# feiyeha/EGM-Unet

Measured on AMD Instinct MI355X. Metric: train images/sec at 3x512x512 bs=8/GPU, higher is better.
Workload: dtype bf16; 1 GPU; EGM-UNet GRFBUNet(3,2,base_c=32) fwd+5-term-loss+bwd+SGD, 8x3x512x512 per GPU (BASELINE.json configs[1]); global_batch=8, parallelism=dp1, launch=hipGraph replay, world_size=1

## Files before the change

### egm_unet_amd/csrc/mca.hip

```cpp
#include "common.h"
#include "bn_elem.h"
#include <stdlib.h>

namespace {

inline int stream_grid(long long total_threads) {
    long long b = (total_threads + 255) / 256;
    if (b > 256 * 16) b = 256 * 16;
    if (b < 1) b = 1;
    return (int)b;
}
__device__ __forceinline__ float sigm(float v) { return 1.f / (1.f + expf(-v)); }

template <typename T, int MODE>
__global__ __launch_bounds__(256) void mca_reduce_row_kernel(const T* __restrict__ a, int lda, const T* __restrict__ b, int ldb,
                                                             float* __restrict__ sums, float* __restrict__ colp, float* __restrict__ chp,
                                                             int H, int W, int C, const float* __restrict__ scale = nullptr,
                                                             const float* __restrict__ shift = nullptr, int act = 0,
                                                             T* __restrict__ zout = nullptr, int ldz = 0) {
    __shared__ float st[2 * 256 * 8];
    __shared__ float red[16];
    const int n = blockIdx.y, h = blockIdx.x, tid = threadIdx.x, ncv = C >> 3, slots = 256 / ncv;
    const int cv = tid % ncv, slot = tid / ncv, L = H + W + C;
    const long long rowbase = ((long long)n * H + h) * W;
    float s8[8], q8[8], ts = 0.f, tq = 0.f;
    zero8(s8); zero8(q8);
    float sc8[8], sh8[8];
    if (MODE == 2) {
#pragma unroll
        for (int j = 0; j < 8; ++j) { sc8[j] = scale[cv * 8 + j]; sh8[j] = shift[cv * 8 + j]; }
    }
    for (int w0 = 0; w0 < W; w0 += slots) {
        const int w = w0 + slot;
        float ps = 0.f, pq = 0.f;
        if (w < W) {
            float v[8];
            load8(a + (rowbase + w) * lda + cv * 8, v);
            if (MODE == 1) {
                float u[8];
                load8(b + (rowbase + w) * ldb + cv * 8, u);
#pragma unroll
                for (int j = 0; j < 8; ++j) v[j] *= u[j];
            }
            if (MODE == 2) {
#pragma unroll
                for (int j = 0; j < 8; ++j) v[j] = to_f32(from_f32<T>(bn_fwd_elem<sizeof(T) == 2>(v[j], sc8[j], sh8[j], act)));
                store8(zout + (rowbase + w) * ldz + cv * 8, v);
            }
#pragma unroll
            for (int j = 0; j < 8; ++j) { s8[j] += v[j]; q8[j] += v[j] * v[j]; ps += v[j]; pq += v[j] * v[j]; }
        }
        ts += ps; tq += pq;
        for (int o = ncv >> 1; o > 0; o >>= 1) { ps += __shfl_xor(ps, o, 64); pq += __shfl_xor(pq, o, 64); }
        if (w < W && cv == 0) { colp[(rowbase + w) * 2 + 0] = ps; colp[(rowbase + w) * 2 + 1] = pq; }
    }
#pragma unroll
    for (int j = 0; j < 8; ++j) { st[tid * 8 + j] = s8[j]; st[(256 + tid) * 8 + j] = q8[j]; }
    __syncthreads();
    for (int c = tid; c < C; c += 256) {
        float cs = 0.f, cq = 0.f;
        for (int sl = 0; sl < slots; ++sl) { cs += st[(sl * ncv + (c >> 3)) * 8 + (c & 7)]; cq += st[(256 + sl * ncv + (c >> 3)) * 8 + (c & 7)]; }
        chp[(((long long)n * H + h) * C + c) * 2 + 0] = cs;
        chp[(((long long)n * H + h) * C + c) * 2 + 1] = cq;
    }
    ts = block_sum(ts, red);
    tq = block_sum(tq, red);
    if (tid == 0) { sums[((long long)n * L + h) * 2 + 0] = ts; sums[((long long)n * L + h) * 2 + 1] = tq; }
}
__global__ __launch_bounds__(256) void mca_reduce_h_kernel(const float* __restrict__ colp, const float* __restrict__ chp, float* __restrict__ sums,
                                                           int N, int H, int W, int C) {
    __shared__ double red[256];
    const int L = H + W + C, per_img = (W + C) * 2;
    const int n = blockIdx.y, col = threadIdx.x & 15, hl = threadIdx.x >> 4;
    const int f = blockIdx.x * 16 + col;
    double s = 0.0;
    if (f < per_img) {
        const bool is_col = f < W * 2;
        const float* src = is_col ? colp + (long long)n * H * W * 2 + f : chp + (long long)n * H * C * 2 + (f - W * 2);
        const int pitch = is_col ? W * 2 : C * 2;
        for (int h = hl; h < H; h += 16) s += (double)src[(long long)h * pitch];
    }
    red[threadIdx.x] = s;
    __syncthreads();
    if (hl == 0 && f < per_img) {
        double t = 0.0;
        for (int j = 0; j < 16; ++j) t += red[j * 16 + col];
        sums[((long long)n * L + H) * 2 + f] = (float)t;
    }
}

struct GateParams {
    const float* w[3];
    const float* k[3];
    int ks[3];
    float inv;
};
__device__ __forceinline__ void axis_of(int e, int H, int W, int C, int& ax, int& idx, int& len) {
    const int L = H + W + C, r = e % L;
    if (r < H) { ax = 0; idx = r; len = H; } else if (r < H + W) { ax = 1; idx = r - H; len = W; } else { ax = 2; idx = r - H - W; len = C; }
}
__device__ __forceinline__ float axis_count(int ax, int H, int W, int C) {
    return ax == 0 ? (float)C * (float)W : (ax == 1 ? (float)C * (float)H : (float)H * (float)W);
}
template <bool LDS_O>
__global__ void mca_gates_fwd_kernel(const float* __restrict__ sums, GateParams gp, float* __restrict__ stats, float* __restrict__ o,
                                     float* __restrict__ gates, int N, int H, int W, int C) {
    extern __shared__ float gate_lds[];
    const int L = H + W + C, total = N * L;
    __shared__ float sk[3][8], sab[3][2];
    if (threadIdx.x < 24) { const int a = threadIdx.x >> 3, t = threadIdx.x & 7; sk[a][t] = t < gp.ks[a] ? gp.k[a][t] : 0.f; }
    else if (threadIdx.x >= 32 && threadIdx.x < 38) { const int a = (threadIdx.x - 32) >> 1, j = (threadIdx.x - 32) & 1; sab[a][j] = gp.ks[a] > 0 ? 0.5f + sigm(gp.w[a][j]) : 0.f; }
    __syncthreads();
    for (int e = threadIdx.x; e < total; e += blockDim.x) {
        int ax, idx, len; axis_of(e, H, W, C, ax, idx, len);
        const double cnt = (double)axis_count(ax, H, W, C);
        const double S = sums[e * 2], Q = sums[e * 2 + 1];
        const double mean = S / cnt;
        double var = (Q - S * S / cnt) / (cnt - 1.0);
        if (var < 0.0) var = 0.0;
        const float sd = (float)sqrt(var);
        stats[e * 2] = (float)mean; stats[e * 2 + 1] = sd;
        const float ov = sab[ax][0] * (float)mean + sab[ax][1] * sd;
        o[e] = ov;
        if (LDS_O) gate_lds[e] = ov;
    }
    __syncthreads();
    const float* os = LDS_O ? gate_lds : o;
    for (int e = threadIdx.x; e < total; e += blockDim.x) {
        int ax, idx, len; axis_of(e, H, W, C, ax, idx, len);
        const int ks = gp.ks[ax], pad = (ks - 1) / 2;
        float z = 0.f;
        for (int t = 0; t < ks; ++t) { const int j = idx + t - pad; if (j >= 0 && j < len) z += sk[ax][t] * os[e - idx + j]; }
        gates[e] = ks > 0 ? sigm(z) : 0.f;
    }
}
template <bool LDS_IN>
__global__ void mca_gates_bwd_kernel(const float* __restrict__ dG, const float* __restrict__ stats, const float* __restrict__ o,
                                     const float* __restrict__ gates, GateParams gp, float* __restrict__ dz, float* __restrict__ coef,
                                     float* __restrict__ dwts, float* __restrict__ dks, int N, int H, int W, int C) {
    extern __shared__ float gate_lds[];
    const int L = H + W + C, total = N * L;
    if (LDS_IN) {
        float* sdz = gate_lds; float* so = gate_lds + total; float* sst = gate_lds + 2 * total;
        for (int e = threadIdx.x; e < total; e += blockDim.x) {
            sdz[e] = dG[e * 2] * gp.inv * gates[e] * (1.f - gates[e]);
            so[e] = o[e];
            sst[2 * e] = stats[2 * e]; sst[2 * e + 1] = stats[2 * e + 1];
        }
        dz = sdz; o = so; stats = sst;
    }
    __shared__ float sk[3][8], sab[3][2];
    if (threadIdx.x < 24) { const int a = threadIdx.x >> 3, t = threadIdx.x & 7; sk[a][t] = t < gp.ks[a] ? gp.k[a][t] : 0.f; }
    else if (threadIdx.x >= 32 && threadIdx.x < 38) { const int a = (threadIdx.x - 32) >> 1, j = (threadIdx.x - 32) & 1; sab[a][j] = gp.ks[a] > 0 ? 0.5f + sigm(gp.w[a][j]) : 0.f; }
    if (threadIdx.x >= 64 && threadIdx.x < 64 + 24) dks[threadIdx.x - 64] = 0.f;
    if (!LDS_IN)
        for (int e = threadIdx.x; e < total; e += blockDim.x) dz[e] = dG[e * 2] * gp.inv * gates[e] * (1.f - gates[e]);
    __syncthreads();
    float acc[27];
#pragma unroll
    for (int i = 0; i < 27; ++i) acc[i] = 0.f;
    for (int e = threadIdx.x; e < total; e += blockDim.x) {
        int ax, idx, len; axis_of(e, H, W, C, ax, idx, len);
        const int ks = gp.ks[ax], pad = (ks - 1) / 2;
        float d_o = 0.f;
        for (int t = 0; t < ks; ++t) { const int i = idx - t + pad; if (i >= 0 && i < len) d_o += sk[ax][t] * dz[e - idx + i]; }
        const float alpha = sab[ax][0], beta = sab[ax][1];
        const float mean = stats[e * 2], sd = stats[e * 2 + 1];
        const float cnt = axis_count(ax, H, W, C);
        const float dmean = alpha * d_o, dsd = beta * d_o;
        const float B = sd > 0.f ? dsd / ((cnt - 1.f) * sd) : 0.f;
        coef[e * 2] = dmean / cnt - B * mean; coef[e * 2 + 1] = B;
        const float dze = dz[e];
#pragma unroll
        for (int a = 0; a < 3; ++a)
            if (a == ax) {
                acc[a * 2] += d_o * mean; acc[a * 2 + 1] += d_o * sd;
#pragma unroll
                for (int t = 0; t < 7; ++t) {
                    const int j = idx + t - pad;
                    if (t < ks && j >= 0 && j < len) acc[6 + a * 7 + t] += dze * o[e - idx + j];
                }
            }
    }
    __shared__ float part[16][27];
    const int lane = threadIdx.x & 63, wv = threadIdx.x >> 6, nw = (blockDim.x + 63) >> 6;
#pragma unroll
    for (int i = 0; i < 27; ++i) { const float v = wave_sum(acc[i]); if (lane == 0) part[wv][i] = v; }
    __syncthreads();
    if (threadIdx.x < 27) {
        float v = 0.f;
        for (int w = 0; w < nw; ++w) v += part[w][threadIdx.x];
        const int i = threadIdx.x;
        if (i < 6) {
            const float sg = gp.ks[i >> 1] > 0 ? sigm(gp.w[i >> 1][i & 1]) : 0.f;
            dwts[i] = v * sg * (1.f - sg);
        } else {
            const int a = (i - 6) / 7, t = (i - 6) % 7;
            if (t < gp.ks[a]) dks[a * 8 + t] = v;
        }
    }
}

template <typename T>
__global__ void mca_xout_kernel(const T* __restrict__ x, int ldx, const float* __restrict__ gates, T* __restrict__ xo, int ldo, int N, int H,
                                int W, int C, float inv) {
    const int ncv = C >> 3, L = H + W + C;
    const long long total = (long long)N * H * W * ncv;
    for (long long i = blockIdx.x * 256LL + threadIdx.x; i < total; i += (long long)gridDim.x * 256) {
        long long p; int cv; egm_divmod(i, ncv, p, cv);
        int w, h, n; egm_pix_nyx(p, H, W, n, h, w);
        const float* g = gates + (long long)n * L;
        const float ghw = g[h] + g[H + w];
        float v[8];
        load8(x + p * ldx + cv * 8, v);
#pragma unroll
        for (int j = 0; j < 8; ++j) v[j] *= (ghw + g[H + W + cv * 8 + j]) * inv;
        store8(xo + p * ldo + cv * 8, v);
    }
}
__device__ __forceinline__ int shuffle_src(int c, int C) { return (c & 3) * (C >> 2) + (c >> 2); }
__device__ __forceinline__ int shuffle_dst(int c, int C) { const int q = C >> 2; return (c % q) * 4 + c / q; }

template <typename T>
__global__ void mca_stencil1_kernel(const T* __restrict__ xo, int ld, T* __restrict__ r1, int ldr, T* __restrict__ u2, int ldu,
                                    unsigned char* __restrict__ codes, int N, int H, int W, int C) {
    const int ncv = C >> 3;
    const long long total = (long long)N * H * W * ncv;
    for (long long i = blockIdx.x * 256LL + threadIdx.x; i < total; i += (long long)gridDim.x * 256) {
        long long p; int cv; egm_divmod(i, ncv, p, cv);
        int xx, yy; egm_pix_yx(p, H, W, yy, xx);
        float c[8], mx[8], mn[8], s[8], v[8];
        int amx[8], amn[8];
        load8(xo + p * ld + cv * 8, c);
#pragma unroll
        for (int j = 0; j < 8; ++j) { mx[j] = -INFINITY; mn[j] = INFINITY; s[j] = 0.f; amx[j] = 4; amn[j] = 4; }
#pragma unroll
        for (int r = -1; r <= 1; ++r)
#pragma unroll
            for (int q = -1; q <= 1; ++q) {
                if (yy + r < 0 || yy + r >= H || xx + q < 0 || xx + q >= W) continue;
                load8(xo + (p + (long long)r * W + q) * ld + cv * 8, v);
#pragma unroll
                for (int j = 0; j < 8; ++j) {
                    if (v[j] > mx[j]) { mx[j] = v[j]; amx[j] = (r + 1) * 3 + (q + 1); }
                    if (v[j] < mn[j]) { mn[j] = v[j]; amn[j] = (r + 1) * 3 + (q + 1); }
                    s[j] += v[j];
                }
            }
        float o1[8], o2[8];
#pragma unroll
        for (int j = 0; j < 8; ++j) {
            const float sh = to_f32(xo[p * ld + shuffle_src(cv * 8 + j, C)]);
            o1[j] = 0.51f * c[j] + 0.2f * (mx[j] - mn[j]) + 0.1f * sh;
            const float u = c[j] - s[j] * (1.f / 9.f);
            o2[j] = u * u;
        }
        store8(r1 + p * ldr + cv * 8, o1); store8(u2 + p * ldu + cv * 8, o2);
        if (codes != nullptr) {
            uint2 cd;
            cd.x = (amx[0] | (amn[0] << 4)) | ((amx[1] | (amn[1] << 4)) << 8) | ((amx[2] | (amn[2] << 4)) << 16) | ((amx[3] | (amn[3] << 4)) << 24);
            cd.y = (amx[4] | (amn[4] << 4)) | ((amx[5] | (amn[5] << 4)) << 8) | ((amx[6] | (amn[6] << 4)) << 16) | ((amx[7] | (amn[7] << 4)) << 24);
            *reinterpret_cast<uint2*>(codes + p * C + cv * 8) = cd;
        }
    }
}
template <typename T>
__global__ void add_avg3_kernel(const T* __restrict__ a, int lda, const T* __restrict__ b, int ldb, float scale, T* __restrict__ out, int ldo,
                                int N, int H, int W, int C) {
    const int ncv = C >> 3;
    const long long total = (long long)N * H * W * ncv;
    for (long long i = blockIdx.x * 256LL + threadIdx.x; i < total; i += (long long)gridDim.x * 256) {
        long long p; int cv; egm_divmod(i, ncv, p, cv);
        int xx, yy; egm_pix_yx(p, H, W, yy, xx);
        float c[8], s[8], v[8];
        load8(a + p * lda + cv * 8, c);
        zero8(s);
#pragma unroll
        for (int r = -1; r <= 1; ++r)
#pragma unroll
            for (int q = -1; q <= 1; ++q) {
                if (yy + r < 0 || yy + r >= H || xx + q < 0 || xx + q >= W) continue;
                load8(b + (p + (long long)r * W + q) * ldb + cv * 8, v);
#pragma unroll
                for (int j = 0; j < 8; ++j) s[j] += v[j];
            }
#pragma unroll
        for (int j = 0; j < 8; ++j) c[j] += scale * s[j] * (1.f / 9.f);
        store8(out + p * ldo + cv * 8, c);
    }
}
constexpr int MF_TY = 16, MF_TX = 16, MF_CB = 32, MF_PY = MF_TY + 4, MF_PX = MF_TX + 4, MF_UY = MF_TY + 2, MF_UX = MF_TX + 2;
template <typename T>
__global__ __launch_bounds__(256) void mca_fused_fwd_kernel(const T* __restrict__ x, int ldx, const float* __restrict__ gates,
                                                            T* __restrict__ xo, int ldxo, T* __restrict__ out, int ldo,
                                                            unsigned char* __restrict__ codes, int N, int H, int W, int C, int tiles_x,
                                                            int tiles_y, int nchunk, float inv) {
    extern __shared__ __attribute__((aligned(16))) unsigned char mf_smem[];
    T* sxo = reinterpret_cast<T*>(mf_smem);
    T* su2 = sxo + MF_PY * MF_PX * MF_CB;
    const int tid = threadIdx.x, L = H + W + C;
    int b = xcd_contiguous_item(blockIdx.x, gridDim.x);
    const int chunk = b % nchunk; b /= nchunk;
    const int tx = b % tiles_x; b /= tiles_x;
    const int ty = b % tiles_y; const int n = b / tiles_y;
    const int y0 = ty * MF_TY, x0 = tx * MF_TX, c0 = chunk * MF_CB;
    const int nvec = (C - c0 < MF_CB ? C - c0 : MF_CB) >> 3;
    const float* __restrict__ g = gates + (long long)n * L;
    const long long img = (long long)n * H * W;
    __shared__ float sgh[MF_PY], sgw[MF_PX];
    if (tid < MF_PY) { const int gy = y0 + tid - 2; sgh[tid] = (gy >= 0 && gy < H) ? g[gy] : 0.f; }
    else if (tid >= 64 && tid < 64 + MF_PX) { const int gx = x0 + tid - 64 - 2; sgw[tid - 64] = (gx >= 0 && gx < W) ? g[H + gx] : 0.f; }
    const int vt = tid & 3;
    float gc8[8], gs8[8];
#pragma unroll
    for (int j = 0; j < 8; ++j) {
        const bool okv = vt < nvec;
        gc8[j] = okv ? g[H + W + c0 + vt * 8 + j] : 0.f;
        gs8[j] = okv ? g[H + W + shuffle_src(c0 + vt * 8 + j, C)] : 0.f;
    }

    constexpr int NC = MF_TY * MF_TX * 4 / 256;
    T shv[NC][8];
#pragma unroll
    for (int k = 0; k < NC; ++k) {
        const int i = tid + k * 256, pix = i >> 2, v = i & 3, ly = pix / MF_TX, lx = pix - ly * MF_TX;
        const int gy = y0 + ly, gx = x0 + lx;
        const bool ok = v < nvec && gy < H && gx < W;
        const long long p = img + (long long)(ok ? gy : 0) * W + (ok ? gx : 0);
        const int q0 = ok ? ((c0 + v * 8) >> 2) : 0;
#pragma unroll
        for (int grp = 0; grp < 4; ++grp) {
            const T* sp = x + p * ldx + (ok ? grp * (C >> 2) : 0) + q0;
            if (sizeof(T) == 2 && ((C >> 2) & 1) == 0) {
                const uint32_t two = *reinterpret_cast<const uint32_t*>(sp);
                __builtin_memcpy(&shv[k][grp], &two, 2);
                const uint16_t hi = (uint16_t)(two >> 16);
                __builtin_memcpy(&shv[k][grp + 4], &hi, 2);
            } else {
                shv[k][grp] = sp[0]; shv[k][grp + 4] = sp[1];
            }
        }
    }
    constexpr int NA = (MF_PY * MF_PX * 4 + 255) / 256;
    uint4 raw[NA];
#pragma unroll
    for (int k = 0; k < NA; ++k) {
        const int i = tid + k * 256, pix = i >> 2, v = i & 3, py = pix / MF_PX, px = pix - py * MF_PX;
        const int gy = y0 + py - 2, gx = x0 + px - 2;
        raw[k] = make_uint4(0, 0, 0, 0);
        if (i < MF_PY * MF_PX * 4 && v < nvec && gy >= 0 && gy < H && gx >= 0 && gx < W) {
            const T* src = x + (img + (long long)gy * W + gx) * ldx + c0 + v * 8;
            if (sizeof(T) == 2) raw[k] = *reinterpret_cast<const uint4*>(src);
        }
    }
    __syncthreads();
#pragma unroll
    for (int k = 0; k < NA; ++k) {
        const int i = tid + k * 256, pix = i >> 2, v = i & 3, py = pix / MF_PX, px = pix - py * MF_PX;
        const int gy = y0 + py - 2, gx = x0 + px - 2;
        if (i >= MF_PY * MF_PX * 4) continue;
        float val[8];
        zero8(val);
        if (v < nvec && gy >= 0 && gy < H && gx >= 0 && gx < W) {
            const long long p = img + (long long)gy * W + gx;
            if (sizeof(T) == 2) load8(reinterpret_cast<const T*>(&raw[k]), val);
            else load8(x + p * ldx + c0 + v * 8, val);
            const float ghw = sgh[py] + sgw[px];
#pragma unroll
            for (int j = 0; j < 8; ++j) val[j] = to_f32(from_f32<T>(val[j] * ((ghw + gc8[j]) * inv)));
            if (xo != nullptr && py >= 2 && py < MF_TY + 2 && px >= 2 && px < MF_TX + 2) store8(xo + p * ldxo + c0 + v * 8, val);
        }
        store8_lds(sxo + pix * MF_CB + v * 8, val);
    }
    __syncthreads();
    for (int i = tid; i < MF_UY * MF_UX * 4; i += 256) {
        const int pix = i >> 2, v = i & 3, uy = pix / MF_UX, ux = pix - uy * MF_UX;
        const int gy = y0 + uy - 1, gx = x0 + ux - 1;
        float o2[8];
        zero8(o2);
        if (v < nvec && gy >= 0 && gy < H && gx >= 0 && gx < W) {
            float c[8], s8[8], t[8];
            zero8(s8);
            const T* ctr = sxo + ((uy + 1) * MF_PX + ux + 1) * MF_CB + v * 8;
            load8(ctr, c);
#pragma unroll
            for (int r = -1; r <= 1; ++r)
#pragma unroll
                for (int q = -1; q <= 1; ++q) {
                    load8(ctr + (r * MF_PX + q) * MF_CB, t);
#pragma unroll
                    for (int j = 0; j < 8; ++j) s8[j] += t[j];
                }
#pragma unroll
            for (int j = 0; j < 8; ++j) { const float u = c[j] - s8[j] * (1.f / 9.f); o2[j] = u * u; }
        }
        store8_lds(su2 + pix * MF_CB + v * 8, o2);
    }
    __syncthreads();
#pragma unroll
    for (int k = 0; k < NC; ++k) {
        const int i = tid + k * 256;
        const int pix = i >> 2, v = i & 3, ly = pix / MF_TX, lx = pix - ly * MF_TX;
        const int gy = y0 + ly, gx = x0 + lx;
        if (v >= nvec || gy >= H || gx >= W) continue;
        const long long p = img + (long long)gy * W + gx;
        float c[8], mx[8], mn[8], t[8], s2[8];
        int amx[8], amn[8];
        const T* ctr = sxo + ((ly + 2) * MF_PX + lx + 2) * MF_CB + v * 8;
        const T* uctr = su2 + ((ly + 1) * MF_UX + lx + 1) * MF_CB + v * 8;
        load8(ctr, c);
        zero8(s2);
#pragma unroll
        for (int j = 0; j < 8; ++j) { mx[j] = -INFINITY; mn[j] = INFINITY; amx[j] = 4; amn[j] = 4; }
#pragma unroll
        for (int r = -1; r <= 1; ++r)
#pragma unroll
            for (int q = -1; q <= 1; ++q) {
                load8(uctr + (r * MF_UX + q) * MF_CB, t);
#pragma unroll
                for (int j = 0; j < 8; ++j) s2[j] += t[j];
                if (gy + r < 0 || gy + r >= H || gx + q < 0 || gx + q >= W) continue;
                load8(ctr + (r * MF_PX + q) * MF_CB, t);
#pragma unroll
                for (int j = 0; j < 8; ++j) {
                    if (t[j] > mx[j]) { mx[j] = t[j]; amx[j] = (r + 1) * 3 + (q + 1); }
                    if (t[j] < mn[j]) { mn[j] = t[j]; amn[j] = (r + 1) * 3 + (q + 1); }
                }
            }
        const float ghw = sgh[ly + 2] + sgw[lx + 2];
        float o[8];
#pragma unroll
        for (int j = 0; j < 8; ++j) {
            const float sh = to_f32(from_f32<T>(to_f32(shv[k][j]) * ((ghw + gs8[j]) * inv)));
            const float o1 = to_f32(from_f32<T>(0.51f * c[j] + 0.2f * (mx[j] - mn[j]) + 0.1f * sh));
            o[j] = o1 + 0.2f * s2[j] * (1.f / 9.f);
        }
        store8(out + p * ldo + c0 + v * 8, o);
        if (codes != nullptr) {
            uint2 cd;
            cd.x = (amx[0] | (amn[0] << 4)) | ((amx[1] | (amn[1] << 4)) << 8) | ((amx[2] | (amn[2] << 4)) << 16) | ((amx[3] | (amn[3] << 4)) << 24);
            cd.y = (amx[4] | (amn[4] << 4)) | ((amx[5] | (amn[5] << 4)) << 8) | ((amx[6] | (amn[6] << 4)) << 16) | ((amx[7] | (amn[7] << 4)) << 24);
            *reinterpret_cast<uint2*>(codes + p * C + c0 + v * 8) = cd;
        }
    }
}
template <typename T>
__global__ void mca_bwd_du_kernel(const T* __restrict__ xo, int ld, const T* __restrict__ g, int ldg, T* __restrict__ du, int ldd, int N, int H,
                                  int W, int C) {
    const int ncv = C >> 3;
    const long long total = (long long)N * H * W * ncv;
    for (long long i = blockIdx.x * 256LL + threadIdx.x; i < total; i += (long long)gridDim.x * 256) {
        long long p; int cv; egm_divmod(i, ncv, p, cv);
        int xx, yy; egm_pix_yx(p, H, W, yy, xx);
        float c[8], s[8], sg[8], v[8];
        load8(xo + p * ld + cv * 8, c);
        zero8(s); zero8(sg);
#pragma unroll
        for (int r = -1; r <= 1; ++r)
#pragma unroll
            for (int q = -1; q <= 1; ++q) {
                if (yy + r < 0 || yy + r >= H || xx + q < 0 || xx + q >= W) continue;
                load8(xo + (p + (long long)r * W + q) * ld + cv * 8, v);
#pragma unroll
                for (int j = 0; j < 8; ++j) s[j] += v[j];
                load8(g + (p + (long long)r * W + q) * ldg + cv * 8, v);
#pragma unroll
                for (int j = 0; j < 8; ++j) sg[j] += v[j];
            }
#pragma unroll
        for (int j = 0; j < 8; ++j) c[j] = 0.4f * (c[j] - s[j] * (1.f / 9.f)) * sg[j] * (1.f / 9.f);
        store8(du + p * ldd + cv * 8, c);
    }
}
template <typename T>
__global__ void mca_bwd_dxo_kernel(const unsigned char* __restrict__ codes, const T* __restrict__ g, int ldg, const T* __restrict__ du, int ldd,
                                   T* __restrict__ dxo, int ldo, int N, int H, int W, int C) {
    const int ncv = C >> 3;
    const long long total = (long long)N * H * W * ncv;
    for (long long i = blockIdx.x * 256LL + threadIdx.x; i < total; i += (long long)gridDim.x * 256) {
        long long p; int cv; egm_divmod(i, ncv, p, cv);
        int xx, yy; egm_pix_yx(p, H, W, yy, xx);
        float acc[8], sd[8], v[8], gp[8];
        zero8(acc); zero8(sd);
#pragma unroll
        for (int r = -1; r <= 1; ++r)
#pragma unroll
            for (int q = -1; q <= 1; ++q) {
                if (yy + r < 0 || yy + r >= H || xx + q < 0 || xx + q >= W) continue;
                const long long pn = p + (long long)r * W + q;
                load8(du + pn * ldd + cv * 8, v);
#pragma unroll
                for (int j = 0; j < 8; ++j) sd[j] += v[j];
                load8(g + pn * ldg + cv * 8, gp);
                const uint2 cd = *reinterpret_cast<const uint2*>(codes + pn * C + cv * 8);
                const int me = (1 - r) * 3 + (1 - q);
#pragma unroll
                for (int j = 0; j < 8; ++j) {
                    const unsigned code = ((j < 4 ? cd.x : cd.y) >> ((j & 3) * 8)) & 0xffu;
                    acc[j] += gp[j] * (((int)(code & 15u) == me ? 1.f : 0.f) - ((int)(code >> 4) == me ? 1.f : 0.f));
                }
            }
        float gc[8], dc[8], o[8];
        load8(g + p * ldg + cv * 8, gc); load8(du + p * ldd + cv * 8, dc);
#pragma unroll
        for (int j = 0; j < 8; ++j) {
            const float gs = to_f32(g[p * ldg + shuffle_dst(cv * 8 + j, C)]);
            o[j] = 0.51f * gc[j] + 0.1f * gs + dc[j] - sd[j] * (1.f / 9.f) + 0.2f * acc[j];
        }
        store8(dxo + p * ldo + cv * 8, o);
    }
}
constexpr int MB_T = 16, MB_CB = 16, MB_P = MB_T + 4, MB_U = MB_T + 2;
template <typename T>
__global__ __launch_bounds__(256) void mca_bwd_fused_kernel(const unsigned char* __restrict__ codes, const T* __restrict__ xo, int ldx,
                                                            const T* __restrict__ g, int ldg, T* __restrict__ dxo, int ldo, int N, int H, int W, int C,
                                                            int tiles_x, int tiles_y, int nchunk) {
    __shared__ __attribute__((aligned(16))) T sxo[MB_P * MB_P * MB_CB];
    __shared__ __attribute__((aligned(16))) T sg[MB_P * MB_P * MB_CB];
    __shared__ __attribute__((aligned(16))) T sdu[MB_U * MB_U * MB_CB];
    __shared__ __attribute__((aligned(16))) unsigned char scd[MB_U * MB_U * MB_CB];
    const int tid = threadIdx.x;
    int b = xcd_contiguous_item(blockIdx.x, gridDim.x);
    const int chunk = b % nchunk; b /= nchunk;
    const int tx = b % tiles_x; b /= tiles_x;
    const int ty = b % tiles_y; const int n = b / tiles_y;
    const int y0 = ty * MB_T, x0 = tx * MB_T, c0 = chunk * MB_CB;
    const int nvec = (C - c0 < MB_CB ? C - c0 : MB_CB) >> 3;
    const long long img = (long long)n * H * W;
    for (int i = tid; i < MB_P * MB_P * 2; i += 256) {
        const int pix = i >> 1, v = i & 1, py = pix / MB_P, px = pix - py * MB_P;
        const int gy = y0 + py - 2, gx = x0 + px - 2;
        uint4 a = make_uint4(0, 0, 0, 0), c = make_uint4(0, 0, 0, 0);
        if (v < nvec && gy >= 0 && gy < H && gx >= 0 && gx < W) {
            const long long p = img + (long long)gy * W + gx;
            a = *reinterpret_cast<const uint4*>(xo + p * ldx + c0 + v * 8);
            c = *reinterpret_cast<const uint4*>(g + p * ldg + c0 + v * 8);
        }
        *reinterpret_cast<uint4*>(sxo + pix * MB_CB + v * 8) = a;
        *reinterpret_cast<uint4*>(sg + pix * MB_CB + v * 8) = c;
    }
    for (int i = tid; i < MB_U * MB_U * 2; i += 256) {
        const int pix = i >> 1, v = i & 1, uy = pix / MB_U, ux = pix - uy * MB_U;
        const int gy = y0 + uy - 1, gx = x0 + ux - 1;
        uint2 cd = make_uint2(0xffffffffu, 0xffffffffu);
        if (v < nvec && gy >= 0 && gy < H && gx >= 0 && gx < W)
            cd = *reinterpret_cast<const uint2*>(codes + (img + (long long)gy * W + gx) * C + c0 + v * 8);
        *reinterpret_cast<uint2*>(scd + pix * MB_CB + v * 8) = cd;
    }
    __syncthreads();
    for (int i = tid; i < MB_U * MB_U * 2; i += 256) {
        const int pix = i >> 1, v = i & 1, uy = pix / MB_U, ux = pix - uy * MB_U;
        const int gy = y0 + uy - 1, gx = x0 + ux - 1;
        float o[8];
        zero8(o);
        if (v < nvec && gy >= 0 && gy < H && gx >= 0 && gx < W) {
            float c[8], s8[8], sg8[8], t[8];
            const T* ctr = sxo + ((uy + 1) * MB_P + ux + 1) * MB_CB + v * 8;
            const T* gtr = sg + ((uy + 1) * MB_P + ux + 1) * MB_CB + v * 8;
            load8(ctr, c);
            zero8(s8); zero8(sg8);
#pragma unroll
            for (int r = -1; r <= 1; ++r)
#pragma unroll
                for (int q = -1; q <= 1; ++q) {
                    load8(ctr + (r * MB_P + q) * MB_CB, t);
#pragma unroll
                    for (int j = 0; j < 8; ++j) s8[j] += t[j];
                    load8(gtr + (r * MB_P + q) * MB_CB, t);
#pragma unroll
                    for (int j = 0; j < 8; ++j) sg8[j] += t[j];
                }
#pragma unroll
            for (int j = 0; j < 8; ++j) o[j] = 0.4f * (c[j] - s8[j] * (1.f / 9.f)) * sg8[j] * (1.f / 9.f);
        }
        store8_lds(sdu + pix * MB_CB + v * 8, o);
    }
    __syncthreads();
    for (int i = tid; i < MB_T * MB_T * 2; i += 256) {
        const int pix = i >> 1, v = i & 1, ly = pix / MB_T, lx = pix - ly * MB_T;
        const int gy = y0 + ly, gx = x0 + lx;
        if (v >= nvec || gy >= H || gx >= W) continue;
        const long long p = img + (long long)gy * W + gx;
        float acc[8], sd[8], t[8], gp[8];
        zero8(acc); zero8(sd);
        const T* dctr = sdu + ((ly + 1) * MB_U + lx + 1) * MB_CB + v * 8;
        const T* gctr = sg + ((ly + 2) * MB_P + lx + 2) * MB_CB + v * 8;
        const unsigned char* cctr = scd + ((ly + 1) * MB_U + lx + 1) * MB_CB + v * 8;
#pragma unroll
        for (int r = -1; r <= 1; ++r)
#pragma unroll
            for (int q = -1; q <= 1; ++q) {
                load8(dctr + (r * MB_U + q) * MB_CB, t);
#pragma unroll
                for (int j = 0; j < 8; ++j) sd[j] += t[j];
                load8(gctr + (r * MB_P + q) * MB_CB, gp);
                const uint2 cd = *reinterpret_cast<const uint2*>(cctr + (r * MB_U + q) * MB_CB);
                const int me = (1 - r) * 3 + (1 - q);
#pragma unroll
                for (int j = 0; j < 8; ++j) {
                    const unsigned code = ((j < 4 ? cd.x : cd.y) >> ((j & 3) * 8)) & 0xffu;
                    acc[j] += gp[j] * (((int)(code & 15u) == me ? 1.f : 0.f) - ((int)(code >> 4) == me ? 1.f : 0.f));
                }
            }
        float gc[8], dc[8], o[8];
        load8(gctr, gc); load8(dctr, dc);
#pragma unroll
        for (int j = 0; j < 8; ++j) {
            const float gs = to_f32(g[p * ldg + shuffle_dst(c0 + v * 8 + j, C)]);
            o[j] = 0.51f * gc[j] + 0.1f * gs + dc[j] - sd[j] * (1.f / 9.f) + 0.2f * acc[j];
        }
        store8(dxo + p * ldo + c0 + v * 8, o);
    }
}
template <typename T>
__global__ void mca_bwd_dx_kernel(const T* __restrict__ dxo, int ldd, const T* __restrict__ x, int ldx, const float* __restrict__ gates,
                                  const float* __restrict__ coef, T* __restrict__ dx, int ldo, int N, int H, int W, int C, float inv) {
    const int ncv = C >> 3, L = H + W + C;
    const long long total = (long long)N * H * W * ncv;
    for (long long i = blockIdx.x * 256LL + threadIdx.x; i < total; i += (long long)gridDim.x * 256) {
        long long p; int cv; egm_divmod(i, ncv, p, cv);
        int w, h, n; egm_pix_nyx(p, H, W, n, h, w);
        const float* g = gates + (long long)n * L;
        const float* cf = coef + (long long)n * L * 2;
        const float ghw = g[h] + g[H + w];
        const float A0 = cf[h * 2] + cf[(H + w) * 2], B0 = cf[h * 2 + 1] + cf[(H + w) * 2 + 1];
        float d[8], v[8];
        load8(dxo + p * ldd + cv * 8, d); load8(x + p * ldx + cv * 8, v);
#pragma unroll
        for (int j = 0; j < 8; ++j) {
            const int c = H + W + cv * 8 + j;
            d[j] = d[j] * (ghw + g[c]) * inv + (A0 + cf[c * 2]) + (B0 + cf[c * 2 + 1]) * v[j];
        }
        store8(dx + p * ldo + cv * 8, d);
    }
}

bool mca_c_ok(int C) { return C >= 8 && C <= 512 && (C & (C - 1)) == 0; }

}

#define EGM_REQ_VEC(name, ptr, ld, C)                                                                      \
    EGM_REQUIRE((ptr) != nullptr && egm_aligned16(ptr) && (C) > 0 && (C) % 8 == 0 && (ld) >= (C) && (ld) % 8 == 0, \
                name ": bad tensor (ptr/alignment/C=%d/ld=%d)", (int)(C), (int)(ld))
#define EGM_REQ_SHAPE(name) EGM_REQUIRE(N > 0 && H > 0 && W > 0, name ": bad shape")
#define EGM_MCA_GRID stream_grid((long long)N * H * W * (C / 8))

extern "C" long long egm_mca_reduce_workspace(int N, int H, int W, int C) {
    if (N <= 0 || H <= 0 || W <= 0 || !mca_c_ok(C)) return -1;
    return ((long long)N * H * W * 2 + (long long)N * H * C * 2) * 4;
}
extern "C" int egm_mca_reduce(int dtype, int mode, const void* a, int lda, const void* b, int ldb, float* sums, void* workspace, int N, int H,
                              int W, int C, egm_stream_t s) {
    EGM_REQ_VEC("mca_reduce", a, lda, C);
    if (mode == 1) EGM_REQ_VEC("mca_reduce", b, ldb, C);
    EGM_REQ_SHAPE("mca_reduce");
    EGM_REQUIRE(sums && workspace && (mode == 0 || mode == 1), "mca_reduce: bad args");
    EGM_REQUIRE(mca_c_ok(C), "mca_reduce: C must be a power of two in [8, 512] (C=%d)", C);
    float* colp = (float*)workspace;
    float* chp = colp + (long long)N * H * W * 2;
    hipStream_t st = (hipStream_t)s;
    EGM_DISPATCH_DTYPE(dtype, {
        if (mode == 0) hipLaunchKernelGGL((mca_reduce_row_kernel<T, 0>), dim3(H, N), dim3(256), 0, st, (const T*)a, lda, (const T*)b, ldb, sums,
                                          colp, chp, H, W, C);
        else hipLaunchKernelGGL((mca_reduce_row_kernel<T, 1>), dim3(H, N), dim3(256), 0, st, (const T*)a, lda, (const T*)b, ldb, sums, colp,
                                chp, H, W, C);
    });
    hipLaunchKernelGGL(mca_reduce_h_kernel, dim3(((W + C) * 2 + 15) / 16, N), dim3(256), 0, st, colp, chp, sums, N, H, W, C);
    EGM_CHECK_LAUNCH("mca_reduce");
    return EGM_OK;
}

extern "C" int egm_mca_reduce_bn(int dtype, const void* y, int ldy, const float* scale, const float* shift, int act, void* z, int ldz,
                                 float* sums, void* workspace, int N, int H, int W, int C, egm_stream_t s) {
    EGM_REQ_VEC("mca_reduce_bn", y, ldy, C);
    EGM_REQ_VEC("mca_reduce_bn", z, ldz, C);
    EGM_REQ_SHAPE("mca_reduce_bn");
    EGM_REQUIRE(sums && workspace && scale && shift, "mca_reduce_bn: bad args");
    EGM_REQUIRE(mca_c_ok(C), "mca_reduce_bn: C must be a power of two in [8, 512] (C=%d)", C);
    float* colp = (float*)workspace;
    float* chp = colp + (long long)N * H * W * 2;
    hipStream_t st = (hipStream_t)s;
    EGM_DISPATCH_DTYPE(dtype, hipLaunchKernelGGL((mca_reduce_row_kernel<T, 2>), dim3(H, N), dim3(256), 0, st, (const T*)y, ldy, (const T*)nullptr,
                                                 0, sums, colp, chp, H, W, C, scale, shift, act, (T*)z, ldz));
    hipLaunchKernelGGL(mca_reduce_h_kernel, dim3(((W + C) * 2 + 15) / 16, N), dim3(256), 0, st, colp, chp, sums, N, H, W, C);
    EGM_CHECK_LAUNCH("mca_reduce_bn");
    return EGM_OK;
}

static int gate_params(GateParams& gp, const float* w_h, const float* k_h, int ks_h, const float* w_w, const float* k_w, int ks_w,
                       const float* w_c, const float* k_c, int ks_c) {
    if (!w_h || !k_h || !w_w || !k_w || (ks_c != 0 && (!w_c || !k_c))) return 0;
    if (ks_h < 1 || ks_h > 7 || ks_w < 1 || ks_w > 7 || ks_c < 0 || ks_c > 7 || !(ks_h & 1) || !(ks_w & 1) || (ks_c != 0 && !(ks_c & 1))) return 0;
    gp.w[0] = w_h; gp.w[1] = w_w; gp.w[2] = w_c; gp.k[0] = k_h; gp.k[1] = k_w; gp.k[2] = k_c; gp.ks[0] = ks_h; gp.ks[1] = ks_w; gp.ks[2] = ks_c;
    gp.inv = ks_c != 0 ? 1.f / 3.f : 0.5f;
    return 1;
}
extern "C" int egm_mca_gates_fwd(const float* sums, const float* w_h, const float* k_h, int ks_h, const float* w_w, const float* k_w,
                                 int ks_w, const float* w_c, const float* k_c, int ks_c, float* stats, float* o, float* gates, int N, int H,
                                 int W, int C, egm_stream_t s) {
    GateParams gp;
    EGM_REQUIRE(gate_params(gp, w_h, k_h, ks_h, w_w, k_w, ks_w, w_c, k_c, ks_c), "mca_gates_fwd: bad gate parameters");
    EGM_REQUIRE(sums && stats && o && gates, "mca_gates_fwd: null pointer");
    EGM_REQ_SHAPE("mca_gates_fwd");
    const size_t lds = (size_t)N * (H + W + C) * sizeof(float);
    if (lds <= 48 * 1024) hipLaunchKernelGGL(mca_gates_fwd_kernel<true>, dim3(1), dim3(1024), lds, (hipStream_t)s, sums, gp, stats, o, gates, N, H, W, C);
    else hipLaunchKernelGGL(mca_gates_fwd_kernel<false>, dim3(1), dim3(1024), 0, (hipStream_t)s, sums, gp, stats, o, gates, N, H, W, C);
    EGM_CHECK_LAUNCH("mca_gates_fwd");
    return EGM_OK;
}
extern "C" int egm_mca_gates_bwd(const float* dG, const float* stats, const float* o, const float* gates, const float* w_h, const float* k_h,
                                 int ks_h, const float* w_w, const float* k_w, int ks_w, const float* w_c, const float* k_c, int ks_c,
                                 float* dz_scratch, float* coef, float* dwts, float* dks, int N, int H, int W, int C, egm_stream_t s) {
    GateParams gp;
    EGM_REQUIRE(gate_params(gp, w_h, k_h, ks_h, w_w, k_w, ks_w, w_c, k_c, ks_c), "mca_gates_bwd: bad gate parameters");
    EGM_REQUIRE(dG && stats && o && gates && dz_scratch && coef && dwts && dks, "mca_gates_bwd: null pointer");
    EGM_REQ_SHAPE("mca_gates_bwd");
    const size_t lds = (size_t)4 * N * (H + W + C) * sizeof(float);
    if (lds <= 140 * 1024) {
        static bool attr_done = false;
        if (!attr_done) {
            hipError_t e = hipFuncSetAttribute(reinterpret_cast<const void*>(mca_gates_bwd_kernel<true>), hipFuncAttributeMaxDynamicSharedMemorySize, 140 * 1024);
            if (e != hipSuccess) EGM_FAIL(EGM_ERR_LAUNCH, "mca_gates_bwd: hipFuncSetAttribute: %s", hipGetErrorString(e));
            attr_done = true;
        }
        hipLaunchKernelGGL(mca_gates_bwd_kernel<true>, dim3(1), dim3(1024), lds, (hipStream_t)s, dG, stats, o, gates, gp, dz_scratch, coef, dwts, dks, N,
                           H, W, C);
    } else {
        hipLaunchKernelGGL(mca_gates_bwd_kernel<false>, dim3(1), dim3(1024), 0, (hipStream_t)s, dG, stats, o, gates, gp, dz_scratch, coef, dwts, dks, N,
                           H, W, C);
    }
    EGM_CHECK_LAUNCH("mca_gates_bwd");
    return EGM_OK;
}
extern "C" int egm_mca_xout(int dtype, const void* x, int ldx, const float* gates, void* xo, int ldo, int N, int H, int W, int C,
                            int no_spatial, egm_stream_t s) {
    const float inv = no_spatial ? 0.5f : 1.f / 3.f;
    EGM_REQ_VEC("mca_xout", x, ldx, C); EGM_REQ_VEC("mca_xout", xo, ldo, C); EGM_REQ_SHAPE("mca_xout");
    EGM_REQUIRE(gates, "mca_xout: null gates");
    EGM_DISPATCH_DTYPE(dtype, hipLaunchKernelGGL((mca_xout_kernel<T>), dim3(EGM_MCA_GRID), dim3(256), 0, (hipStream_t)s, (const T*)x, ldx, gates,
                                                 (T*)xo, ldo, N, H, W, C, inv));
    EGM_CHECK_LAUNCH("mca_xout");
    return EGM_OK;
}
extern "C" int egm_mca_stencil1(int dtype, const void* xo, int ld, void* r1, int ldr, void* u2, int ldu, unsigned char* codes, int N, int H,
                                int W, int C, egm_stream_t s) {
    EGM_REQ_VEC("mca_stencil1", xo, ld, C); EGM_REQ_VEC("mca_stencil1", r1, ldr, C); EGM_REQ_VEC("mca_stencil1", u2, ldu, C);
    EGM_REQ_SHAPE("mca_stencil1");
    EGM_REQUIRE(C % 4 == 0 && (codes == nullptr || (reinterpret_cast<uintptr_t>(codes) & 7) == 0), "mca_stencil1: bad codes buffer");
    EGM_DISPATCH_DTYPE(dtype, hipLaunchKernelGGL((mca_stencil1_kernel<T>), dim3(EGM_MCA_GRID), dim3(256), 0, (hipStream_t)s, (const T*)xo, ld,
                                                 (T*)r1, ldr, (T*)u2, ldu, codes, N, H, W, C));
    EGM_CHECK_LAUNCH("mca_stencil1");
    return EGM_OK;
}
extern "C" int egm_add_avg3(int dtype, const void* a, int lda, const void* b, int ldb, float scale, void* out, int ldo, int N, int H, int W,
                            int C, egm_stream_t s) {
    EGM_REQ_VEC("add_avg3", a, lda, C); EGM_REQ_VEC("add_avg3", b, ldb, C); EGM_REQ_VEC("add_avg3", out, ldo, C); EGM_REQ_SHAPE("add_avg3");
    EGM_DISPATCH_DTYPE(dtype, hipLaunchKernelGGL((add_avg3_kernel<T>), dim3(EGM_MCA_GRID), dim3(256), 0, (hipStream_t)s, (const T*)a, lda,
                                                 (const T*)b, ldb, scale, (T*)out, ldo, N, H, W, C));
    EGM_CHECK_LAUNCH("add_avg3");
    return EGM_OK;
}
// ... 73 lines not shown
```

Before: 687.9 images/s.

## Use packed integer keys for MCA window min/max argmin/argmax in fused forward

Converts the bf16 values in the shared tile into sign-magnitude integer keys with embedded position labels. A 3x3 window min/max together with its argmin/argmax then reduces to integer min3/max3 over row-reduced partials that are reused across vertically adjacent outputs. In the backward pass, the per-element code compares become packed bitwise hit-weight extraction, and the channel-shuffle index division is computed incrementally. This trades extra LDS passes and syncs, plus some register pressure, for far fewer compare and select instructions in the stencil.

```diff
diff --git a/egm_unet_amd/csrc/mca.hip b/egm_unet_amd/csrc/mca.hip
--- a/egm_unet_amd/csrc/mca.hip
+++ b/egm_unet_amd/csrc/mca.hip
@@ -1,6 +1,14 @@
 #include "common.h"
 #include "bn_elem.h"
+#include "mca_keys.h"
+#include <limits.h>
 #include <stdlib.h>
+
+#ifdef EGM_MCA_SCAN
+constexpr bool kMcaKeys = false;
+#else
+constexpr bool kMcaKeys = true;
+#endif
 
 namespace {
 
@@ -220,6 +228,16 @@
 }
 __device__ __forceinline__ int shuffle_src(int c, int C) { return (c & 3) * (C >> 2) + (c >> 2); }
 __device__ __forceinline__ int shuffle_dst(int c, int C) { const int q = C >> 2; return (c % q) * 4 + c / q; }
+__device__ __forceinline__ void shuffle_dst8(int cb, int C, int (&dst)[8]) {
+    const int q = C >> 2;
+    int d = (int)egm_udiv(cb, q), m = cb - d * q;
+#pragma unroll
+    for (int j = 0; j < 8; ++j) {
+        dst[j] = m * 4 + d;
+        const bool wrap = ++m == q;
+        m = wrap ? 0 : m; d += wrap ? 1 : 0;
+    }
+}
 
 template <typename T>
 __global__ void mca_stencil1_kernel(const T* __restrict__ xo, int ld, T* __restrict__ r1, int ldr, T* __restrict__ u2, int ldu,
@@ -290,11 +308,93 @@
     }
 }
 constexpr int MF_TY = 16, MF_TX = 16, MF_CB = 32, MF_PY = MF_TY + 4, MF_PX = MF_TX + 4, MF_UY = MF_TY + 2, MF_UX = MF_TX + 2;
+template <bool BORDER>
+__device__ __forceinline__ void mca_fwd_window_keys(const uint32_t* __restrict__ skey, const bf16_t* __restrict__ su2, const uint4 (&ctr)[4],
+                                                    const uint32_t (&shp)[4][4], const float (&gs8)[8], const float* __restrict__ sgh,
+                                                    const float* __restrict__ sgw, bf16_t* __restrict__ out, int ldo,
+                                                    unsigned char* __restrict__ codes, long long img, int y0, int x0, int c0, int nvec, int H,
+                                                    int W, int C, float inv) {
+    const int tid = threadIdx.x, wv = __builtin_amdgcn_readfirstlane(tid >> 6), lx = (tid >> 2) & 15, v = tid & 3, gx = x0 + lx;
+    const bool dupl = BORDER && gx - 1 < 0, dupr = BORDER && gx + 1 >= W;
+    const bool lane_ok = !BORDER || (v < nvec && gx < W);
+    const uint32_t cl = dupl ? 1u : 0u, cr = dupr ? 1u : 2u;
+    int rmn[6][8], rmx[6][8];
+    auto row = [&](int j) {
+        if (BORDER) {
+            const int gyr = y0 + 4 * wv + j - 1;
+            if (gyr < 0 || gyr >= H) {
+#pragma unroll
+                for (int e = 0; e < 8; ++e) { rmn[j][e] = INT_MAX; rmx[j][e] = INT_MIN; }
+                return;
+            }
+        }
+        const uint32_t* p = skey + (((4 * wv + 1 + j) * MF_PX + lx + 2) * MF_CB + v * 8) / 2;
+        uint4 c4 = *reinterpret_cast<const uint4*>(p), l4 = *reinterpret_cast<const uint4*>(p - MF_CB / 2),
+              r4 = *reinterpret_cast<const uint4*>(p + MF_CB / 2);
+        if (BORDER) { if (dupl) l4 = c4; if (dupr) r4 = c4; }
+        const uint32_t l[4] = {l4.x, l4.y, l4.z, l4.w}, c[4] = {c4.x, c4.y, c4.z, c4.w}, r[4] = {r4.x, r4.y, r4.z, r4.w};
+        const uint32_t nl = mca_min_label(j * 3) + (cl << MCA_LABEL_SHIFT), nc = mca_min_label(j * 3 + 1), nr = mca_min_label(j * 3) + (cr << MCA_LABEL_SHIFT);
+#pragma unroll
+        for (int d = 0; d < 4; ++d) {
+            const int la = mca_word_lo(l[d], nl), ca = mca_word_lo(c[d], nc), ra = mca_word_lo(r[d], nr);
+            const int lb = mca_word_hi(l[d], nl), cb = mca_word_hi(c[d], nc), rb = mca_word_hi(r[d], nr);
+            rmn[j][2 * d] = mca_min3(la, ca, ra);
+            rmn[j][2 * d + 1] = mca_min3(lb, cb, rb);
+            rmx[j][2 * d] = mca_max3(mca_max_word(la), mca_max_word(ca), mca_max_word(ra));
+            rmx[j][2 * d + 1] = mca_max3(mca_max_word(lb), mca_max_word(cb), mca_max_word(rb));
+        }
+    };
+    row(0); row(1);
+#pragma unroll
+    for (int k = 0; k < 4; ++k) {
+        const int ly = 4 * wv + k, gy = y0 + ly;
+        if (BORDER && gy >= H) break;
+        row(k + 2);
+        const long long p = img + (long long)gy * W + gx;
+        float c[8], t[8], s2[8];
+        load8(reinterpret_cast<const bf16_t*>(&ctr[k]), c);
+        const bf16_t* uctr = su2 + ((ly + 1) * MF_UX + lx + 1) * MF_CB + v * 8;
+        zero8(s2);
+#pragma unroll
+        for (int r = -1; r <= 1; ++r)
+#pragma unroll
+            for (int q = -1; q <= 1; ++q) {
+                load8(uctr + (r * MF_UX + q) * MF_CB, t);
+#pragma unroll
+                for (int j = 0; j < 8; ++j) s2[j] += t[j];
+            }
+        const float ghw = sgh[ly + 2] + sgw[lx + 2];
+        float o[8];
+        int wmn[8], wmx[8];
+#pragma unroll
+        for (int j = 0; j < 8; ++j) {
+            wmn[j] = mca_min3(rmn[k][j], rmn[k + 1][j], rmn[k + 2][j]);
+            wmx[j] = mca_max3(rmx[k][j], rmx[k + 1][j], rmx[k + 2][j]);
+            wmn[j] = min(wmn[j], mca_min_sentinel(3 * k + 4));
+            wmx[j] = max(wmx[j], mca_max_sentinel(3 * k + 4));
+            const float mx = __uint_as_float(mca_word_f32_bits(wmx[j])), mn = __uint_as_float(mca_word_f32_bits(wmn[j]));
+            const float sx = __uint_as_float(j < 4 ? shp[k][j] << 16 : shp[k][j - 4] & 0xffff0000u);
+            const float sh = to_f32(from_f32<bf16_t>(sx * ((ghw + gs8[j]) * inv)));
+            const float o1 = to_f32(from_f32<bf16_t>(0.51f * c[j] + 0.2f * (mx - mn) + 0.1f * sh));
+            o[j] = o1 + 0.2f * s2[j] * (1.f / 9.f);
+        }
+        if (lane_ok) {
+            store8(out + p * ldo + c0 + v * 8, o);
+            if (codes != nullptr) {
+                uint2 cd;
+                cd.x = mca_codes4(mca_labels4(wmn[0], wmn[1], wmn[2], wmn[3]), mca_labels4(wmx[0], wmx[1], wmx[2], wmx[3]), 3 * k);
+                cd.y = mca_codes4(mca_labels4(wmn[4], wmn[5], wmn[6], wmn[7]), mca_labels4(wmx[4], wmx[5], wmx[6], wmx[7]), 3 * k);
+                *reinterpret_cast<uint2*>(codes + p * C + c0 + v * 8) = cd;
+            }
+        }
+    }
+}
 template <typename T>
 __global__ __launch_bounds__(256) void mca_fused_fwd_kernel(const T* __restrict__ x, int ldx, const float* __restrict__ gates,
                                                             T* __restrict__ xo, int ldxo, T* __restrict__ out, int ldo,
                                                             unsigned char* __restrict__ codes, int N, int H, int W, int C, int tiles_x,
                                                             int tiles_y, int nchunk, float inv) {
+    constexpr bool KEYS = sizeof(T) == 2 && kMcaKeys;
     extern __shared__ __attribute__((aligned(16))) unsigned char mf_smem[];
     T* sxo = reinterpret_cast<T*>(mf_smem);
     T* su2 = sxo + MF_PY * MF_PX * MF_CB;
@@ -322,7 +422,7 @@
     constexpr int NC = MF_TY * MF_TX * 4 / 256;
     T shv[NC][8];
 #pragma unroll
-    for (int k = 0; k < NC; ++k) {
+    for (int k = 0; k < (KEYS ? 0 : NC); ++k) {
         const int i = tid + k * 256, pix = i >> 2, v = i & 3, ly = pix / MF_TX, lx = pix - ly * MF_TX;
         const int gy = y0 + ly, gx = x0 + lx;
         const bool ok = v < nvec && gy < H && gx < W;
@@ -373,6 +473,22 @@
         store8_lds(sxo + pix * MF_CB + v * 8, val);
     }
     __syncthreads();
+    uint32_t shp[NC][4];
+    if constexpr (KEYS) {
+#pragma unroll
+        for (int k = 0; k < NC; ++k) {
+            const int ly = 4 * (tid >> 6) + k, lx = (tid >> 2) & 15, v = tid & 3, gy = y0 + ly, gx = x0 + lx;
+            const bool ok = v < nvec && gy < H && gx < W;
+            const long long p = img + (long long)(ok ? gy : 0) * W + (ok ? gx : 0);
+            const int q0 = ok ? ((c0 + v * 8) >> 2) : 0;
+#pragma unroll
+            for (int grp = 0; grp < 4; ++grp) {
+                const T* sp = x + p * ldx + (ok ? grp * (C >> 2) : 0) + q0;
+                if (((C >> 2) & 1) == 0) shp[k][grp] = *reinterpret_cast<const uint32_t*>(sp);
+                else shp[k][grp] = (uint32_t)sp[0].v | ((uint32_t)sp[1].v << 16);
+            }
+        }
+    }
     for (int i = tid; i < MF_UY * MF_UX * 4; i += 256) {
         const int pix = i >> 2, v = i & 3, uy = pix / MF_UX, ux = pix - uy * MF_UX;
         const int gy = y0 + uy - 1, gx = x0 + ux - 1;
@@ -395,6 +511,26 @@
             for (int j = 0; j < 8; ++j) { const float u = c[j] - s8[j] * (1.f / 9.f); o2[j] = u * u; }
         }
         store8_lds(su2 + pix * MF_CB + v * 8, o2);
+    }
+    if constexpr (KEYS) {
+        uint4 ctr[NC];
+#pragma unroll
+        for (int k = 0; k < NC; ++k)
+            ctr[k] = *reinterpret_cast<const uint4*>(sxo + ((4 * (tid >> 6) + k + 2) * MF_PX + ((tid >> 2) & 15) + 2) * MF_CB + (tid & 3) * 8);
+        __syncthreads();
+        for (int i = tid; i < MF_UY * MF_UX * 4; i += 256) {
+            const int pix = i >> 2, v = i & 3, uy = pix / MF_UX, ux = pix - uy * MF_UX;
+            uint4* q = reinterpret_cast<uint4*>(sxo + ((uy + 1) * MF_PX + ux + 1) * MF_CB + v * 8);
+            uint4 a = *q;
+            a.x = mca_key2(a.x); a.y = mca_key2(a.y); a.z = mca_key2(a.z); a.w = mca_key2(a.w);
+            *q = a;
+        }
+        __syncthreads();
+        const uint32_t* skey = reinterpret_cast<const uint32_t*>(sxo);
+        const bool interior = y0 >= 1 && y0 + MF_TY + 1 <= H && x0 >= 1 && x0 + MF_TX + 1 <= W && nvec == 4;
+        if (interior) mca_fwd_window_keys<false>(skey, su2, ctr, shp, gs8, sgh, sgw, out, ldo, codes, img, y0, x0, c0, nvec, H, W, C, inv);
+        else mca_fwd_window_keys<true>(skey, su2, ctr, shp, gs8, sgh, sgw, out, ldo, codes, img, y0, x0, c0, nvec, H, W, C, inv);
+        return;
     }
     __syncthreads();
 #pragma unroll
@@ -596,17 +732,29 @@
                 load8(gctr + (r * MB_P + q) * MB_CB, gp);
                 const uint2 cd = *reinterpret_cast<const uint2*>(cctr + (r * MB_U + q) * MB_CB);
                 const int me = (1 - r) * 3 + (1 - q);
-#pragma unroll
-                for (int j = 0; j < 8; ++j) {
-                    const unsigned code = ((j < 4 ? cd.x : cd.y) >> ((j & 3) * 8)) & 0xffu;
-                    acc[j] += gp[j] * (((int)(code & 15u) == me ? 1.f : 0.f) - ((int)(code >> 4) == me ? 1.f : 0.f));
+                if constexpr (sizeof(T) == 2 && kMcaKeys) {
+                    const uint32_t wl = mca_hit_weights4(cd.x, me), wh = mca_hit_weights4(cd.y, me);
+#pragma unroll
+                    for (int j = 0; j < 8; ++j) acc[j] += gp[j] * mca_weight(j < 4 ? wl : wh, j & 3);
+                } else {
+#pragma unroll
+                    for (int j = 0; j < 8; ++j) {
+                        const unsigned code = ((j < 4 ? cd.x : cd.y) >> ((j & 3) * 8)) & 0xffu;
+                        acc[j] += gp[j] * (((int)(code & 15u) == me ? 1.f : 0.f) - ((int)(code >> 4) == me ? 1.f : 0.f));
+                    }
                 }
             }
         float gc[8], dc[8], o[8];
         load8(gctr, gc); load8(dctr, dc);
+        int dst[8];
+        if constexpr (sizeof(T) == 2 && kMcaKeys) shuffle_dst8(c0 + v * 8, C, dst);
+        else {
+#pragma unroll
+            for (int j = 0; j < 8; ++j) dst[j] = shuffle_dst(c0 + v * 8 + j, C);
+        }
 #pragma unroll
         for (int j = 0; j < 8; ++j) {
-            const float gs = to_f32(g[p * ldg + shuffle_dst(c0 + v * 8 + j, C)]);
+            const float gs = to_f32(g[p * ldg + dst[j]]);
             o[j] = 0.51f * gc[j] + 0.1f * gs + dc[j] - sd[j] * (1.f / 9.f) + 0.2f * acc[j];
         }
         store8(dxo + p * ldo + c0 + v * 8, o);
diff --git a/egm_unet_amd/csrc/mca_keys.h b/egm_unet_amd/csrc/mca_keys.h
--- /dev/null
+++ b/egm_unet_amd/csrc/mca_keys.h
@@ -0,0 +1,53 @@
+#pragma once
+#include <stdint.h>
+
+#if defined(__HIPCC__) || defined(__CUDACC__)
+#define MCA_KEYS_FN __host__ __device__ static inline
+#else
+#define MCA_KEYS_FN static inline
+#endif
+
+constexpr int MCA_LABEL_SHIFT = 8;
+constexpr uint32_t MCA_ELEMENT_FLAG = 0x4000u;
+constexpr int MCA_LABEL_TOP = 31;
+
+MCA_KEYS_FN int mca_key(uint32_t bf16_bits) {
+    const int s = (int)(int16_t)(uint16_t)bf16_bits, a = s & 0x7fff;
+    return s < 0 ? -a : a;
+}
+MCA_KEYS_FN uint32_t mca_key_bits(int key) { return key < 0 ? (0x8000u | (uint32_t)(-key)) : (uint32_t)key; }
+
+MCA_KEYS_FN uint32_t mca_key2(uint32_t two_bf16) {
+    return ((uint32_t)mca_key(two_bf16 & 0xffffu) & 0xffffu) | ((uint32_t)mca_key(two_bf16 >> 16) << 16);
+}
+MCA_KEYS_FN int mca_word_lo(uint32_t two_keys, uint32_t label_field) { return (int)((two_keys << 16) | label_field); }
+MCA_KEYS_FN int mca_word_hi(uint32_t two_keys, uint32_t label_field) { return (int)((two_keys & 0xffff0000u) | label_field); }
+MCA_KEYS_FN uint32_t mca_min_label(int scan_index) { return MCA_ELEMENT_FLAG | ((uint32_t)scan_index << MCA_LABEL_SHIFT); }
+MCA_KEYS_FN int mca_max_word(int min_word) { return min_word ^ (MCA_LABEL_TOP << MCA_LABEL_SHIFT); }
+MCA_KEYS_FN int mca_min_sentinel(int centre) { return (int)((0x7f80u << 16) | ((uint32_t)centre << MCA_LABEL_SHIFT)); }
+MCA_KEYS_FN int mca_max_sentinel(int centre) { return (int)(((uint32_t)-0x7f80 << 16) | 0x8000u | ((uint32_t)(MCA_LABEL_TOP - centre) << MCA_LABEL_SHIFT)); }
+
+MCA_KEYS_FN int mca_min3(int a, int b, int c) { const int m = a < b ? a : b; return m < c ? m : c; }
+MCA_KEYS_FN int mca_max3(int a, int b, int c) { const int m = a > b ? a : b; return m > c ? m : c; }
+
+MCA_KEYS_FN uint32_t mca_word_f32_bits(int word) {
+    const uint32_t hi = (uint32_t)word & 0xffff0000u;
+    return word < 0 ? 0x80000000u - hi : hi;
+}
+MCA_KEYS_FN uint32_t mca_labels4(int w0, int w1, int w2, int w3) {
+    return (((uint32_t)w0 >> 8) & 0xffu) | ((uint32_t)w1 & 0xff00u) | (((uint32_t)w2 << 8) & 0xff0000u) | (((uint32_t)w3 << 16) & 0xff000000u);
+}
+MCA_KEYS_FN uint32_t mca_codes4(uint32_t min_labels4, uint32_t max_labels4, int first) {
+    const uint32_t amn = (min_labels4 & 0x1f1f1f1fu) - 0x01010101u * (uint32_t)first;
+    const uint32_t amx = 0x01010101u * (uint32_t)(MCA_LABEL_TOP - first) - (max_labels4 & 0x1f1f1f1fu);
+    return amx | (amn << 4);
+}
+
+MCA_KEYS_FN uint32_t mca_hit_weights4(uint32_t codes4, int me) {
+    const uint32_t w = codes4 ^ (0x11111111u * (uint32_t)me);
+    const uint32_t nz = ((w & 0x77777777u) + 0x77777777u) | w;
+    const uint32_t mxm = (nz >> 3) & 0x01010101u, mnm = (nz >> 7) & 0x01010101u;
+    const uint32_t one = mxm ^ mnm, neg = one & mxm;
+    return one + ((neg << 8) - (neg << 1));
+}
+MCA_KEYS_FN float mca_weight(uint32_t weights4, int j) { return (float)(int)(int8_t)(uint8_t)(weights4 >> (8 * j)); }
```

Measured after the change: 694.3 images/s (median of 6 runs). About the same (+0.9%).
